# daac-tools/daachorse

Hardware: AMD Instinct MI355X
Metric: haystack GB/s scanned (find_overlapping_iter(..).count(), 100k-pattern bytewise automaton) (higher is better)
Workload: dtype u8/u32 integer

## Files before the change

### daachorse_amd/csrc/gram4_kernels.hip

```cpp
#include <hip/hip_runtime.h>

#include <algorithm>
#include <cstdint>
#include <utility>

#include "device_tables.hpp"
#include "gram4_filter.hpp"
#include "gram4_index.hpp"

namespace daac {

namespace {

typedef uint32_t g4_u32x4_t __attribute__((ext_vector_type(4)));
constexpr uint32_t kList4 = 256;
constexpr uint32_t kProbePercent4 = 3;
typedef __attribute__((address_space(3))) const uint32_t lds4_cu32;
typedef __attribute__((address_space(3))) uint32_t lds4_u32;
typedef __attribute__((address_space(3))) const uint16_t lds4_cu16;
typedef __attribute__((address_space(3))) uint16_t lds4_u16;
typedef __attribute__((address_space(3))) const uint8_t lds4_cu8;
typedef __attribute__((address_space(3))) g4_u32x4_t lds4_u32x4;

__device__ __forceinline__ uint32_t pin4(uint32_t x) {
    asm("" : "+v"(x));
    return x;
}
__device__ __forceinline__ uint32_t mad24(uint32_t a, uint32_t b, uint32_t c) {
    uint32_t d;
    asm("v_mad_u32_u24 %0, %1, %2, %3" : "=v"(d) : "v"(a), "s"(b), "v"(c));
    return d;
}
__device__ __forceinline__ uint32_t wave_shr1_4(uint32_t v, uint32_t lane0) {
    uint32_t d = lane0;
    asm volatile("s_nop 1\nv_mov_b32_dpp %0, %1 wave_shr:1 row_mask:0xf bank_mask:0xf" : "+v"(d) : "v"(v));
    return d;
}
__device__ __forceinline__ uint32_t g4_wave_scan(uint32_t v) {
    v += static_cast<uint32_t>(__builtin_amdgcn_update_dpp(0, static_cast<int>(v), 0x111, 0xf, 0xf, false));
    v += static_cast<uint32_t>(__builtin_amdgcn_update_dpp(0, static_cast<int>(v), 0x112, 0xf, 0xf, false));
    v += static_cast<uint32_t>(__builtin_amdgcn_update_dpp(0, static_cast<int>(v), 0x114, 0xf, 0xf, false));
    v += static_cast<uint32_t>(__builtin_amdgcn_update_dpp(0, static_cast<int>(v), 0x118, 0xf, 0xf, false));
    v += static_cast<uint32_t>(__builtin_amdgcn_update_dpp(0, static_cast<int>(v), 0x142, 0xa, 0xf, false));
    v += static_cast<uint32_t>(__builtin_amdgcn_update_dpp(0, static_cast<int>(v), 0x143, 0xc, 0xf, false));
    return v;
}
template <typename F, int... I>
__device__ __forceinline__ void g4_turns(F &&f, std::integer_sequence<int, I...>) {
    (void)(... && f(std::integral_constant<int, I>{}));
}
__device__ __forceinline__ unsigned long long g4_wave_sum(unsigned long long v) {
#pragma unroll
    for (int off = 32; off > 0; off >>= 1) v += __shfl_down(v, off, 64);
    return v;
}
__device__ __forceinline__ void g4_copy(void *dst, const void *src, uint32_t bytes) {
    const uint4 *s = reinterpret_cast<const uint4 *>(src);
    uint4 *d = reinterpret_cast<uint4 *>(dst);
    for (uint32_t i = threadIdx.x; i < bytes / 16; i += blockDim.x) d[i] = s[i];
}
__device__ __forceinline__ void g4_reduce(unsigned long long cnt, unsigned long long *scratch, unsigned long long *result) {
    const unsigned long long c = g4_wave_sum(cnt);
    __syncthreads();
    const int wave = threadIdx.x >> 6, lane = threadIdx.x & 63;
    if (lane == 0) scratch[wave] = c;
    __syncthreads();
    if (threadIdx.x == 0) {
        unsigned long long r0 = 0;
        for (int w = 0; w < static_cast<int>((blockDim.x + 63) >> 6); ++w) r0 += scratch[w];
        if (r0) atomicAdd(result, r0);
    }
}

}

template <int K, int Q, bool ARITH, int DIR, bool TAIL, bool FILT, bool MPH = false>
__device__ __forceinline__ void gram4_body(const Gram4Dev &g, const GramArgs &a, const Gram4Lds &L, char *smem) {
    static_assert(!(FILT && TAIL), "the filter runs in front of the plain records");
    static_assert(!(FILT && DIR == 0), "the filter's Bloom array lies where the per-word directory would");
    static_assert(!MPH || FILT, "the perfect hash serves the survivors of the filter");
    constexpr int P = 16 * Q;
    constexpr int GS = 8;
    constexpr uint32_t SB = 64u * P;
    constexpr uint32_t SLOT = SB + 32u;
    const uint32_t offM = L.off_m, offS = L.off_s, offC = L.off_cls;
    const uint32_t lo = g.lo, OTH = g.C - 1u, C = g.C;
    auto cls_of = [&](uint32_t byte) -> uint32_t {
        if (ARITH) {
            const uint32_t u = byte - lo;
            return u < OTH ? u : OTH;
        }
        return *reinterpret_cast<lds4_cu8 *>(static_cast<uintptr_t>(offC + byte));
    };
    auto lds_u32 = [&](uint32_t addr) -> uint32_t { return *reinterpret_cast<lds4_cu32 *>(static_cast<uintptr_t>(addr)); };
    auto below = [&](uint32_t k) -> uint32_t { return (1u << k) - 1u; };

    const uint32_t lane = threadIdx.x & 63;
    const uint32_t lane_off = pin4(lane * (16u * Q));
    const uint32_t wave_in_wg = __builtin_amdgcn_readfirstlane(threadIdx.x >> 6);
    const uint32_t C4 = C * 4u, CC4 = C * C * 4u;
    const uint32_t offM1 = g4i_off1(offM, C);
    const uint32_t ub4 = g.unused_byte * 0x01010101u;
    const uint8_t *__restrict__ hay = a.hay_al;
    const uint64_t nwaves = static_cast<uint64_t>(gridDim.x) * (blockDim.x >> 6);
    const uint32_t tb = L.off_wave + wave_in_wg * L.wave_stride;
    const uint32_t listb = wave_in_wg * (kList4 * 2u);
    const uint64_t slab_index = (static_cast<uint64_t>(blockIdx.x) * (blockDim.x >> 6) + wave_in_wg) * a.wq_slab;
    uint4 *__restrict__ slab4 = reinterpret_cast<uint4 *>(a.wq) + slab_index;
    uint32_t wq_n = 0, slab_hi = 0;
    uint64_t epoch_base = 0;
    const uint32_t drain_early = wave_in_wg * 64u;

    unsigned long long tot_cnt = 0;
    uint32_t cnt32 = 0;

    auto load_chunk = [&](uint64_t v) -> uint4 {
        if (v >= a.vlen) return uint4{ub4, ub4, ub4, ub4};
        const g4_u32x4_t q = __builtin_nontemporal_load(reinterpret_cast<const g4_u32x4_t *>(hay + v));
        uint4 r{q.x, q.y, q.z, q.w};
        if (v < a.lead || v + 16 > a.vlen) {
            uint32_t w[4] = {r.x, r.y, r.z, r.w};
            for (int b = 0; b < 16; ++b) {
                const uint64_t p = v + b;
                if (p < a.lead || p >= a.vlen) w[b >> 2] = (w[b >> 2] & ~(0xffu << (8 * (b & 3)))) | (g.unused_byte << (8 * (b & 3)));
            }
            r = uint4{w[0], w[1], w[2], w[3]};
        }
        return r;
    };
    auto raw_at = [&](uint64_t p) -> uint32_t { return (p >= a.lead && p < a.vlen) ? hay[p] : g.unused_byte; };
    auto read_ahead = [&](uint64_t v) -> unsigned long long {
        unsigned long long x;
        if (v >= a.lead && v + 8 <= a.vlen) {
            __builtin_memcpy(&x, hay + v, 8);
        } else {
            x = 0;
            for (int b = 7; b >= 0; --b) x = (x << 8) | ((v + b >= a.lead && v + b < a.vlen) ? hay[v + b] : g.unused_byte);
        }
        return x;
    };
    auto tail_count = [&](const uint4 &rr, unsigned long long text) -> uint32_t {
        const uint32_t edges = rr.x & 15u;
        const unsigned long long path = (static_cast<unsigned long long>(rr.w) << 32) | rr.z;
        const unsigned long long diff = path ^ text;
        uint32_t same = diff ? static_cast<uint32_t>(__builtin_ctzll(diff)) >> 3 : 8u;
        same = same < edges ? same : edges;
        return __popc((rr.x >> 4) & ((2u << same) - 1u) & 0x1ffu);
    };
    auto drain = [&]() {
        const uint4 *__restrict__ recs = TAIL ? g.drec_t : g.drec_c;
        uint32_t n_in = wq_n;
        bool raw = !TAIL;
        while (n_in != 0) {
            uint32_t n_out = 0;
            for (uint32_t base = 0; base < n_in; base += 64u) {
                const uint32_t i = base + lane;
                const bool live = i < n_in;
                uint4 e = uint4{0u, 0u, 0u, 0u};
                if (live) e = slab4[i];
                uint32_t state, n_ahead, pos = e.x;
                unsigned long long ah;
                if (raw) {
                    const uint32_t k1 = cls_of(e.w & 0xffu);
                    state = e.y + __popc(e.x & below(k1));
                    pos = e.z;
                    ah = e.w >> 8;
                    n_ahead = 3;
                } else {
                    state = e.y & 0x07ffffffu;
                    ah = (static_cast<unsigned long long>(e.w & 0xffffffu) << 32) | e.z;
                    n_ahead = e.w >> 24;
                }
                uint4 rr = uint4{0u, 0u, 0u, 0u};
                if (live) rr = recs[state];
                const uint64_t vn = epoch_base + pos + 2;
                bool cont = false;
                uint32_t next_state = 0;
                if (rr.x >> 31) {
                    if (n_ahead < (rr.x & 15u)) ah = read_ahead(vn);
                    cnt32 += tail_count(rr, ah);
                } else {
                    if (live && n_ahead == 0u) { ah = read_ahead(vn); n_ahead = 8; }
                    const uint32_t k = cls_of(static_cast<uint32_t>(ah) & 0xffu);
                    cnt32 += rr.z;
                    cont = ((rr.x >> k) & 1u) != 0;
                    next_state = rr.y + __popc(rr.x & below(k));
                }
                const unsigned long long m = __ballot(cont);
                if (m != 0) {
                    if (cont) {
                        const uint32_t at = n_out + __builtin_amdgcn_mbcnt_hi(static_cast<uint32_t>(m >> 32), __builtin_amdgcn_mbcnt_lo(static_cast<uint32_t>(m), 0));
                        ah >>= 8;
                        slab4[at] = uint4{pos + 1u, next_state, static_cast<uint32_t>(ah), static_cast<uint32_t>(ah >> 32) | ((n_ahead - 1u) << 24)};
                    }
                    n_out += static_cast<uint32_t>(__popcll(m));
                }
            }
            n_in = n_out;
            raw = false;
        }
        wq_n = 0;
    };

    uint32_t q_head = 0, q_tail = 0;
    uint32_t posbias = 0;
    uint32_t st_n = 0;
    uint32_t pend_lo = 0;
    uint4 pend = uint4{0u, 0u, 0u, 0u};
    uint32_t pend_pos = 0;
    uint32_t pend_t0 = 0, pend_t1 = 0;
    bool pend_valid = false;
    uint4 p2 = uint4{0u, 0u, 0u, 0u};
    uint32_t p2_pos = 0, p2_state = 0;
    uint32_t p2_t0 = 0, p2_t1 = 0;
    bool p2_live = false, p2_any = false;
    uint32_t sb_n = 0;
    uint32_t sb_pos = 0, sb_lo = 0, sb_t0 = 0;
    uint32_t fp_pos = 0, fp_t0 = 0;
    const uint32_t offB = L.off_b, bloomW = g.bloom_words;
    auto push_walker = [&](bool go, const uint4 &entry) {
        const unsigned long long m = __ballot(go);
        if (m != 0) {
            if (go) {
                const uint32_t at = wq_n + __builtin_amdgcn_mbcnt_hi(static_cast<uint32_t>(m >> 32), __builtin_amdgcn_mbcnt_lo(static_cast<uint32_t>(m), 0));
                slab4[at] = entry;
            }
            wq_n += __popcll(m);
        }
    };
    auto finish_second = [&]() {
        if (!TAIL || !p2_any) return;
        p2_any = false;
        const uint4 r = p2;
        bool again = false;
        uint32_t st_k = 0, pos = p2_pos, t0 = p2_t0, t1n = (p2_t1 & 0xffffffu) | (7u << 24);
        if (p2_live) {
            if (r.x >> 31) {
                if ((r.x & 15u) <= 7u) cnt32 += tail_count(r, (static_cast<unsigned long long>(p2_t1) << 32) | p2_t0);
                else { again = true; st_k = p2_state; }
            } else {
                cnt32 += r.z;
                const uint32_t k = p2_state >> 27;
                if ((r.x >> k) & 1u) {
                    again = true;
                    const uint32_t k3 = cls_of((p2_t0 >> 8) & 0xffu);
                    st_k = (r.y + __popc(r.x & below(k))) | (k3 << 27);
                    pos = p2_pos + 1u;
                    t0 = __builtin_amdgcn_alignbyte(p2_t1, p2_t0, 1u);
                    t1n = ((p2_t1 >> 8) & 0xffffu) | (6u << 24);
                }
            }
        }
        p2_live = false;
        push_walker(again, uint4{pos, st_k, t0, t1n});
    };
    auto consume_pending = [&]() {
        finish_second();
        if (!pend_valid) return;
        pend_valid = false;
        const uint4 r = pend;
        if (FILT) {
            const uint32_t k1 = cls_of(fp_t0 & 0xffu);
            cnt32 += (r.x >> kGram4EndsBitDev) & 1u;
            push_walker(__builtin_amdgcn_ubfe(r.x, k1, 1) != 0, uint4{r.x, r.y, fp_pos, fp_t0});
            return;
        }
        const uint32_t k1 = cls_of(pend_t0 & 0xffu);
        if (!TAIL) {
            cnt32 += (r.x >> kGram4EndsBitDev) & 1u;
            push_walker(__builtin_amdgcn_ubfe(r.x, k1, 1) != 0, uint4{r.x, r.y, pend_pos, pend_t0});
            return;
        }
        bool go;
        if (r.x >> 31) {
            cnt32 += tail_count(r, (static_cast<unsigned long long>(pend_t1) << 32) | pend_t0);
            go = false;
        } else {
            cnt32 += (r.x >> kGram4EndsBitDev) & 1u;
            go = ((r.x >> k1) & 1u) != 0;
        }
        p2 = uint4{0u, 0u, 0u, 0u};
        p2_live = go;
        p2_any = __ballot(go) != 0;
        if (go) {
            const uint32_t child = r.y + __popc(r.x & below(k1));
            const uint32_t k2 = cls_of((pend_t0 >> 8) & 0xffu);
            p2 = g.drec_t[child];
            p2_pos = pend_pos;
            p2_state = child | (k2 << 27);
            p2_t0 = __builtin_amdgcn_alignbyte(pend_t1, pend_t0, 1u);
            p2_t1 = pend_t1 >> 8;
        }
    };
    auto derive = [&](uint32_t first, uint32_t cnt) {
        if (lane - first < cnt) {
            const uint32_t t3 = *reinterpret_cast<lds4_cu16 *>(static_cast<uintptr_t>(listb + ((q_head + lane - first) << 1)));
            pend_pos = t3 + posbias;
            const uint32_t a0 = t3 & ~3u, sh = t3 & 3u;
            const uint32_t d0 = lds_u32(a0), d1 = lds_u32(a0 + 4u), d2 = lds_u32(a0 + 8u);
            pend_lo = __builtin_amdgcn_alignbyte(d1, d0, sh);
            pend_t0 = __builtin_amdgcn_alignbyte(d2, d1, sh);
            if (TAIL) {
                const uint32_t d3 = lds_u32(a0 + 12u);
                pend_t1 = __builtin_amdgcn_alignbyte(d3, d2, sh);
            }
        }
        q_head += cnt;
    };
    const uint32_t lo_idx = K == 3 ? lo * (C * C + C + 1u) : lo * (C + 1u);
    auto rank_and_ask = [&](uint32_t x_lo) {
        uint32_t idx, d;
        if (ARITH) {
            idx = mad24((x_lo >> 8) & 0xffu, C, ((x_lo >> 16) & 0xffu) - lo_idx);
            if (K == 3) idx = mad24(x_lo & 0xffu, C * C, idx);
            d = (x_lo >> 24) - lo;
        } else {
            const uint32_t c1 = cls_of((x_lo >> 8) & 0xffu), c2 = cls_of((x_lo >> 16) & 0xffu);
            d = cls_of(x_lo >> 24);
            idx = __umul24(c1, C) + c2;
            if (K == 3) idx = __umul24(cls_of(x_lo & 0xffu), C * C) + idx;
        }
        const uint32_t am = (idx << 2) + offM;
        const uint32_t own = lds_u32(am);
        uint32_t rank;
        if (DIR == 0) {
            const uint32_t base = *reinterpret_cast<lds4_cu16 *>(static_cast<uintptr_t>((idx << 1) + offS));
            rank = base + __popc(own & below(d));
        } else {
            const uint32_t grp = am & ~15u;
            const uint32_t qx = lds_u32(grp), qy = lds_u32(grp + 4u), qz = lds_u32(grp + 8u);
            const uint32_t gi = pin4(idx >> 2);
            const uint32_t base = DIR == 1 ? *reinterpret_cast<lds4_cu16 *>(static_cast<uintptr_t>((gi << 1) + offS))
                                           : *reinterpret_cast<lds4_cu32 *>(static_cast<uintptr_t>((gi << 2) + offS));
            const uint32_t mx = static_cast<uint32_t>(__builtin_amdgcn_sbfe(static_cast<int>(0xEEEEEEEEu), idx, 1u));
            const uint32_t my = static_cast<uint32_t>(__builtin_amdgcn_sbfe(static_cast<int>(0xCCCCCCCCu), idx, 1u));
            const uint32_t mz = static_cast<uint32_t>(__builtin_amdgcn_sbfe(static_cast<int>(0x88888888u), idx, 1u));
            uint32_t under = __popc(own & below(d));
            under += __popc(qx & mx & 0x3fffffffu);
            under += __popc(qy & my & 0x3fffffffu);
            under += __popc(qz & mz & 0x3fffffffu);
            rank = base + under;
        }
        if (TAIL) {
            pend = g.dhit_t[rank];
        } else {
            const uint2 h = g.dhit_c[rank];
            pend = uint4{h.x, h.y, 0u, 0u};
        }
    };
    const G4Mph mph = g.mph;
    auto hash_and_ask = [&](uint32_t x_lo) {
        const uint32_t x = K == 3 ? x_lo : x_lo >> 8;
        const uint32_t h = g4f_h(x);
        const uint32_t d = *reinterpret_cast<lds4_cu8 *>(static_cast<uintptr_t>(offS + g4m_bucket(h, mph)));
        const uint2 r = g.dhit_h[g4m_slot(h, g4m_f(x, mph), d, mph)];
        pend = uint4{r.x, r.y, 0u, 0u};
    };
    auto survivors_ask = [&](uint32_t n) {
        consume_pending();
        pend = uint4{0u, 0u, 0u, 0u};
        if (lane < n) { if constexpr (MPH) hash_and_ask(sb_lo); else rank_and_ask(sb_lo); }
        fp_pos = sb_pos;
        fp_t0 = lane < n ? sb_t0 : 0u;
        pend_valid = true;
    };
    auto process_batch = [&](uint32_t n) {
        __builtin_amdgcn_s_setprio(2);
        if (FILT) {
            derive(st_n, n - st_n);
            st_n = 0;
            const G4Probe pr = g4f_probe(K == 3 ? pend_lo : pend_lo >> 8, pend_t0 & 0xffu, bloomW);
            const uint32_t fw = lds_u32(offB + (pr.word << 2));
            const unsigned long long in_batch = n >= 64u ? ~0ull : (1ull << n) - 1ull;
            const unsigned long long pm = (__builtin_amdgcn_ballot_w64((pr.go & ~fw) == 0u) | __builtin_amdgcn_ballot_w64((pr.ends & ~fw) == 0u)) & in_batch;
            if (pm != 0) {
                const uint32_t s = static_cast<uint32_t>(__popcll(pm));
                const uint32_t r = __builtin_amdgcn_mbcnt_hi(static_cast<uint32_t>(pm >> 32), __builtin_amdgcn_mbcnt_lo(static_cast<uint32_t>(pm), 0));
                uint32_t t;
                asm("v_cndmask_b32_e64 %0, 63, %1, %2" : "=v"(t) : "v"(r), "s"(pm));
                const uint32_t tgt = ((t + sb_n) << 2) & 0xfcu;
                const uint32_t r_pos = static_cast<uint32_t>(__builtin_amdgcn_ds_permute(static_cast<int>(tgt), static_cast<int>(pend_pos)));
                const uint32_t r_lo = static_cast<uint32_t>(__builtin_amdgcn_ds_permute(static_cast<int>(tgt), static_cast<int>(pend_lo)));
                const uint32_t r_t0 = static_cast<uint32_t>(__builtin_amdgcn_ds_permute(static_cast<int>(tgt), static_cast<int>(pend_t0)));
                const bool mine = lane - sb_n < s;
                sb_pos = mine ? r_pos : sb_pos;
                sb_lo = mine ? r_lo : sb_lo;
                sb_t0 = mine ? r_t0 : sb_t0;
                if (sb_n + s >= 64u) {
                    survivors_ask(64u);
                    sb_pos = r_pos; sb_lo = r_lo; sb_t0 = r_t0;
                    sb_n = sb_n + s - 64u;
                } else {
                    sb_n += s;
                }
            }
            return;
        }
        consume_pending();
        derive(st_n, n - st_n);
        st_n = 0;
        pend = uint4{0u, 0u, 0u, 0u};
        if (lane < n) {
            rank_and_ask(pend_lo);
        } else {
            pend_t0 = 0;
            pend_t1 = 0;
        }
        pend_valid = true;
    };

    uint64_t region = static_cast<uint64_t>(blockIdx.x) * (blockDim.x >> 6) + wave_in_wg;
    while (region < a.nregions) {
      slab_hi = static_cast<uint32_t>((region * a.region_bytes) >> 31);
      epoch_base = static_cast<uint64_t>(slab_hi) << 31;
      for (; region < a.nregions && static_cast<uint32_t>((region * a.region_bytes) >> 31) == slab_hi; region += nwaves) {
        const uint64_t rbase = region * a.region_bytes;
        const uint64_t rend = rbase + a.region_bytes < a.vlen ? rbase + a.region_bytes : a.vlen;
        uint32_t carry = 0, tail4 = 0;
#pragma unroll
        for (int i = 0; i < K; ++i) carry |= (rbase >= static_cast<uint64_t>(K - i) ? cls_of(raw_at(rbase - (K - i))) : OTH) << (8 * i);
#pragma unroll
        for (int i = 0; i < 4; ++i) tail4 |= (rbase >= static_cast<uint64_t>(4 - i) ? raw_at(rbase - (4 - i)) : static_cast<uint32_t>(g.unused_byte)) << (8 * i);
        tail4 = __builtin_amdgcn_readfirstlane(tail4);
        carry = __builtin_amdgcn_readfirstlane(carry);
        uint32_t mcarry;
        {
            uint32_t x = (((carry >> (8 * (K - 1))) & 0xffu) << 2) + offM;
            x += __umul24((carry >> (8 * (K - 2))) & 0xffu, C4);
            if (K == 3) x += __umul24(carry & 0xffu, CC4);
            mcarry = __builtin_amdgcn_readfirstlane(lds_u32(x));
        }

        const uint32_t rlen = static_cast<uint32_t>(rend - rbase);
        const uint32_t fast_lo = rbase < 16u ? SB : 0u;
        const uint32_t fast_hi = rlen & ~(SB - 1u);
        auto fetch = [&](uint32_t off, uint4 (&out)[Q]) {
            if (off >= fast_lo && off < fast_hi) {
                const uint8_t *__restrict__ base = hay + rbase + off;
                uint32_t voff = lane_off;
                asm volatile("" : "+v"(voff));
#pragma unroll
                for (int q = 0; q < Q; ++q) {
                    const g4_u32x4_t t = __builtin_nontemporal_load(reinterpret_cast<const g4_u32x4_t *>(base + voff + 16u * q));
                    out[q] = uint4{t.x, t.y, t.z, t.w};
                }
                return;
            }
            const uint64_t s0 = rbase + off;
#pragma unroll
            for (int q = 0; q < Q; ++q) out[q] = uint4{ub4, ub4, ub4, ub4};
            if (off < rlen) {
#pragma unroll
                for (int q = 0; q < Q; ++q) out[q] = load_chunk(s0 + lane * P + 16u * q);
            } else if (lane == 0 && off < rlen + SB) {
                out[0] = load_chunk(s0);
            }
        };
        uint4 pf0[Q], pf1[Q];
        fetch(0u, pf0);
        fetch(SB, pf1);
        const uint32_t rbias = static_cast<uint32_t>(rbase - epoch_base) - (tb + 16u - 3u);

        for (uint32_t off = 0; off < rlen; off += SB) {
            if (wq_n + 64u * P + 128u + drain_early > a.wq_slab) drain();
            uint4 cur[Q];
#pragma unroll
            for (int q = 0; q < Q; ++q) { cur[q] = pf0[q]; pf0[q] = pf1[q]; }
            consume_pending();
            __builtin_amdgcn_s_setprio(0);
            fetch(off + 2u * SB, pf1);

            if (q_tail != q_head) {
                const uint32_t n_left = q_tail - q_head;
                derive(st_n, n_left);
                st_n += n_left;
            }
            q_head = q_tail = 0;
            const uint32_t slot = tb;
            const uint32_t my_text = slot + 16u + lane * P;
            posbias = rbias + off;
#pragma unroll
            for (int q = 0; q < Q; ++q)
                *reinterpret_cast<lds4_u32x4 *>(static_cast<uintptr_t>(my_text + 16u * q)) = g4_u32x4_t{cur[q].x, cur[q].y, cur[q].z, cur[q].w};
            if (lane == 0) {
                *reinterpret_cast<lds4_u32 *>(static_cast<uintptr_t>(slot + 12u)) = tail4;
                *reinterpret_cast<lds4_u32x4 *>(static_cast<uintptr_t>(slot + 16u + SB)) = g4_u32x4_t{pf0[0].x, pf0[0].y, pf0[0].z, pf0[0].w};
            }
            tail4 = __builtin_amdgcn_readlane(cur[Q - 1].w, 63);

            uint32_t kx[K + P];
#pragma unroll
            for (int q = 0; q < Q; ++q) {
                const uint32_t w[4] = {cur[q].x, cur[q].y, cur[q].z, cur[q].w};
#pragma unroll
                for (int b = 0; b < 16; ++b) {
                    kx[K + 16 * q + b] = pin4(cls_of((w[b >> 2] >> (8 * (b & 3))) & 0xffu));
                    __builtin_assume(kx[K + 16 * q + b] < 32u);
                }
            }
            uint32_t pk = 0;
#pragma unroll
            for (int i = 0; i < K; ++i) pk |= kx[P + i] << (8 * i);
            const uint32_t left = wave_shr1_4(pk, carry);
            carry = __builtin_amdgcn_readlane(pk, 63);
#pragma unroll
            for (int i = 0; i < K; ++i) { kx[i] = (left >> (8 * i)) & 0xffu; __builtin_assume(kx[i] < 32u); }

            uint32_t H = 0, ccnt = cnt32, roll = 0, mprev = 0;
#pragma unroll
            for (int grp = 0; grp < P / GS; ++grp) {
                uint32_t mw[GS];
                uint32_t qe = 0;
#pragma unroll
                for (int jj = 0; jj < GS; ++jj) {
                    const int j = grp * GS + jj;
                    uint32_t x;
                    if (K == 3 && (jj & 1)) {
                        x = g4i_odd(qe, kx[K + j], offM1, C);
                    } else if (K == 3) {
                        const G4Idx e = g4i_even(kx[K + j], kx[K + j - 1], kx[K + j - 2], offM, C);
                        x = e.addr;
                        qe = e.q;
                    } else {
                        x = pin4((kx[K + j] << 2) + offM);
                        x = mad24(kx[K + j - 1], C4, x);
                    }
                    mw[jj] = lds_u32(x);
                }
#pragma unroll
                for (int jj = 0; jj < GS; ++jj) {
                    const int j = grp * GS + jj;
                    roll = __builtin_amdgcn_alignbit(roll, mw[jj], 30);
                    if (j > 0) H = __builtin_amdgcn_alignbit((jj == 0 ? mprev : mw[jj - 1]) >> kx[K + j], H, 1);
                    if ((j & 15) == 15) {
                        ccnt = pin4(__popc(roll) + ccnt);
                        ccnt = pin4(__popc(roll & 0xaaaaaaaau) + ccnt);
                        roll = 0;
                    }
                }
                mprev = mw[GS - 1];
            }
            {
                const uint32_t mleft = wave_shr1_4(mprev, mcarry);
                mcarry = __builtin_amdgcn_readlane(mprev, 63);
                H |= __builtin_amdgcn_ubfe(mleft, kx[K], 1) << (32 - P);
            }
            cnt32 = ccnt;

            static_assert(P == 16 * Q, "lane_off = lane * 16 Q is this lane's offset in the step: my_text = tb + 16 + lane_off");
            const uint32_t text_adj = tb + (lane_off - (32u - P) + 13u);
            for (;;) {
                if (__ballot(H != 0u) == 0) break;
                const uint32_t n = __popc(H);
                const uint32_t incl = g4_wave_scan(n);
                const uint32_t tot = __builtin_amdgcn_readlane(incl, 63);
                const uint32_t first = q_tail + incl - n;
                const uint32_t room = first < kList4 ? kList4 - first : 0u;
                const uint32_t lim = n < room ? n : room;
                const uint32_t at = pin4(listb + (first << 1));
                g4_turns([&](auto tc) -> bool {
                    constexpr uint32_t t = decltype(tc)::value;
                    const bool w = t < lim;
                    if (__ballot(w) == 0) return false;
                    if (w) {
                        *reinterpret_cast<lds4_u16 *>(static_cast<uintptr_t>(at + 2u * t)) = static_cast<uint16_t>(text_adj + __builtin_ctz(H));
                        H &= H - 1u;
                    }
                    return true;
                }, std::make_integer_sequence<int, P>{});
                const uint32_t in = std::min(tot, kList4 - q_tail);
                q_tail += in;
                while (st_n + q_tail - q_head >= 64u) process_batch(64u);
                if (in == tot) break;
                const uint32_t n_left = q_tail - q_head;
                if (lane < n_left) {
                    const uint16_t v = *reinterpret_cast<lds4_cu16 *>(static_cast<uintptr_t>(listb + ((q_head + lane) << 1)));
                    *reinterpret_cast<lds4_u16 *>(static_cast<uintptr_t>(listb + (lane << 1))) = v;
                }
                q_head = 0;
                q_tail = n_left;
            }
        }
        tot_cnt += cnt32;
        cnt32 = 0;
      }
      if (st_n + q_tail - q_head != 0) process_batch(st_n + q_tail - q_head);
      if (FILT && sb_n != 0) { survivors_ask(sb_n); sb_n = 0; }
      consume_pending();
      finish_second();
      drain();
      tot_cnt += cnt32;
      cnt32 = 0;
    }
    g4_reduce(tot_cnt, reinterpret_cast<unsigned long long *>(smem), a.result);
}

template <int K, int Q, bool ARITH, int DIR, int TPB, bool FILT, bool MPH = false>
__global__ __launch_bounds__(TPB) void gram4_kernel(const Gram4Dev g, const GramArgs a, const Gram4Lds L) {
    extern __shared__ __attribute__((aligned(16))) char smem[];
    constexpr int DIRC = DIR == 0 ? 1 : DIR;
    if (!ARITH) g4_copy(smem + L.off_cls, g.cls, 256);
    g4_copy(smem + L.off_m, g.m, g.m_bytes);
    uint32_t *votes = reinterpret_cast<uint32_t *>(smem + L.off_wave);
    if (threadIdx.x == 0) *votes = 0;
    __syncthreads();
    if (__builtin_amdgcn_groupstaticsize() != 0) __builtin_trap();
    bool tail = a.sel_want == 1u;
    if (a.sel_want == 2u) {
        const uint64_t span = a.vlen > a.lead + 16 ? a.vlen - a.lead - 8 : 0;
        bool go = false;
        if (span != 0) {
            unsigned long long h = (static_cast<unsigned long long>(threadIdx.x) + 1) * 0x9E3779B97F4A7C15ull;
            h ^= h >> 29;
            const uint64_t p = a.lead + 3 + (h % (span - 3));
            const uint8_t *t = a.hay_al + p;
            const uint32_t OTH = g.C - 1u;
            auto cl = [&](uint32_t b) -> uint32_t {
                if (ARITH) { const uint32_t u = b - g.lo; return u < OTH ? u : OTH; }
                return reinterpret_cast<const uint8_t *>(smem + L.off_cls)[b];
            };
            const uint32_t *m = reinterpret_cast<const uint32_t *>(smem + L.off_m);
            const uint32_t c0 = cl(t[-3]), c1 = cl(t[-2]), c2 = cl(t[-1]), d = cl(t[0]), k1 = cl(t[1]);
            const uint32_t ctx = K == 3 ? (c0 * g.C + c1) * g.C + c2 : c1 * g.C + c2;
            const uint32_t w = m[ctx];
            if ((w >> d) & 1u & (d < OTH ? 1u : 0u)) {
                uint32_t rank = __popc(w & ((1u << d) - 1u));
                for (uint32_t j = ctx & ~3u; j < ctx; ++j) rank += __popc(m[j] & 0x3fffffffu);
                rank += g.s16 ? reinterpret_cast<const uint16_t *>(g.sdir)[ctx >> 2] : reinterpret_cast<const uint32_t *>(g.sdir)[ctx >> 2];
                const uint2 r = g.dhit_c[rank];
                go = ((r.x >> k1) & 1u) != 0;
            }
        }
        const unsigned long long bm = __ballot(go);
        if ((threadIdx.x & 63) == 0 && bm != 0) atomicAdd(votes, static_cast<uint32_t>(__popcll(bm)));
        __syncthreads();
        tail = *votes * 100u > static_cast<uint32_t>(TPB) * kProbePercent4;
        __syncthreads();
    }
    if (FILT && !tail) {
        g4_copy(smem + L.off_s, MPH ? static_cast<const void *>(g.mph_disp) : g.sdir, L.s_bytes_f);
        g4_copy(smem + L.off_b, g.bloom, g.bloom_words * 4u);
    } else {
        g4_copy(smem + L.off_s, DIR == 0 ? static_cast<const void *>(g.rfull) : g.sdir, L.s_bytes);
    }
    __syncthreads();
    if (tail) gram4_body<K, Q, ARITH, DIR, true, false>(g, a, L, smem);
    else if constexpr (FILT) gram4_body<K, Q, ARITH, DIRC, false, true, MPH>(g, a, L, smem);
    else gram4_body<K, Q, ARITH, DIR, false, false>(g, a, L, smem);
}

template <int K, int Q, bool ARITH, int DIR, int TPB, bool FILT, bool MPH = false>
static hipError_t launch4_inst(const Gram4Dev &dev, const GramArgs &a, const Gram4Lds &L, uint32_t blocks, hipStream_t stream) {
    const hipError_t e = hipFuncSetAttribute(reinterpret_cast<const void *>(gram4_kernel<K, Q, ARITH, DIR, TPB, FILT, MPH>),
                                             hipFuncAttributeMaxDynamicSharedMemorySize, static_cast<int>(L.lds_bytes));
    if (e != hipSuccess) return e;
    hipLaunchKernelGGL((gram4_kernel<K, Q, ARITH, DIR, TPB, FILT, MPH>), dim3(blocks), dim3(TPB), L.lds_bytes, stream, dev, a, L);
    return hipGetLastError();
}
template <int K, int Q, int TPB, bool ARITH>
static hipError_t launch4_d(const Gram4Dev &dev, const GramArgs &a, const Gram4Lds &L, uint32_t blocks, hipStream_t stream) {
    if (L.filter && L.mph) {
        if (L.dir == 0) return launch4_inst<K, Q, ARITH, 0, TPB, true, true>(dev, a, L, blocks, stream);
        if (L.dir == 1) return launch4_inst<K, Q, ARITH, 1, TPB, true, true>(dev, a, L, blocks, stream);
        return launch4_inst<K, Q, ARITH, 2, TPB, true, true>(dev, a, L, blocks, stream);
    }
    if (L.filter) {
        if (L.dir == 0) return launch4_inst<K, Q, ARITH, 0, TPB, true>(dev, a, L, blocks, stream);
        if (L.dir == 1) return launch4_inst<K, Q, ARITH, 1, TPB, true>(dev, a, L, blocks, stream);
        return launch4_inst<K, Q, ARITH, 2, TPB, true>(dev, a, L, blocks, stream);
    }
    if (L.dir == 0) return launch4_inst<K, Q, ARITH, 0, TPB, false>(dev, a, L, blocks, stream);
    if (L.dir == 1) return launch4_inst<K, Q, ARITH, 1, TPB, false>(dev, a, L, blocks, stream);
    return launch4_inst<K, Q, ARITH, 2, TPB, false>(dev, a, L, blocks, stream);
}
template <int K, int Q, int TPB>
static hipError_t launch4_k(const Gram4Dev &dev, const GramArgs &a, const Gram4Lds &L, uint32_t blocks, hipStream_t stream) {
    return L.arith ? launch4_d<K, Q, TPB, true>(dev, a, L, blocks, stream) : launch4_d<K, Q, TPB, false>(dev, a, L, blocks, stream);
}

bool gram4_plan(const Gram4Dev &dev, uint32_t ppl, uint32_t waves, bool rfull, bool want_arith, bool want_filter, uint32_t lds_limit, Gram4Lds &L) {
    L = Gram4Lds{};
    if (rfull && dev.rfull == nullptr) return false;
    const uint32_t slot = 64u * ppl + 32u;
    L.wave_stride = slot;
    L.off_wave = waves * kList4 * 2u;
    L.threads = waves * 64u;
    L.arith = (want_arith && dev.arith) ? 1u : 0u;
    const uint32_t per_wg = L.off_wave + waves * L.wave_stride;
    L.off_cls = per_wg;
    L.off_s = per_wg + (L.arith ? 0u : 256u);
    L.dir = rfull ? 0u : (dev.s16 ? 1u : 2u);
    L.s_bytes = rfull ? dev.rfull_bytes : dev.s_bytes;
    uint32_t region = L.s_bytes;
    if (want_filter && dev.bloom != nullptr) {
        const uint32_t front = dev.mph_disp != nullptr ? dev.mph_bytes : dev.s_bytes;
        const uint32_t with = front + dev.bloom_words * 4u;
        if (L.off_s + std::max(region, with) + dev.m_bytes <= lds_limit) {
            L.filter = 1u;
            L.mph = dev.mph_disp != nullptr ? 1u : 0u;
            L.s_bytes_f = front;
            L.off_b = L.off_s + front;
            region = std::max(region, with);
        }
    }
    L.off_m = L.off_s + region;
    L.lds_bytes = L.off_m + dev.m_bytes;
    return L.lds_bytes <= lds_limit;
}
uint32_t gram4_filter_room(uint32_t m_bytes, uint32_t sdir_bytes, bool arith, uint32_t lds_limit) {
    const uint32_t fixed = 16u * kList4 * 2u + 16u * (64u * 32u + 32u) + (arith ? 0u : 256u) + sdir_bytes + m_bytes;
    return fixed < lds_limit ? (lds_limit - fixed) & ~15u : 0u;
}

hipError_t launch_gram4_scan(const Gram4Dev &dev, const GramArgs &a, const Gram4Lds &L, uint32_t blocks, hipStream_t stream) {
    if (a.ppl == 32 && L.threads == 1024)
        return dev.K == 3 ? launch4_k<3, 2, 1024>(dev, a, L, blocks, stream) : launch4_k<2, 2, 1024>(dev, a, L, blocks, stream);
    if (a.ppl == 32)
        return dev.K == 3 ? launch4_k<3, 2, 512>(dev, a, L, blocks, stream) : launch4_k<2, 2, 512>(dev, a, L, blocks, stream);
    if (L.threads == 512)
        return dev.K == 3 ? launch4_k<3, 1, 512>(dev, a, L, blocks, stream) : launch4_k<2, 1, 512>(dev, a, L, blocks, stream);
    return dev.K == 3 ? launch4_k<3, 1, 1024>(dev, a, L, blocks, stream) : launch4_k<2, 1, 1024>(dev, a, L, blocks, stream);
}

}
```

Baseline: 1775.

## Drain work queue incrementally with batched multi-row loads and cooked-entry tagging

The drain routine now processes up to DR batches of 64 queue entries at once (three when Q==2), issuing all slab and record loads before consuming them so the memory latencies overlap. In non-tail mode it drains one pass early once the queue passes a per-wave threshold, keeping the sub-64 remainder. Raw and already-advanced entries can now sit in the same queue, so advanced ones are tagged with a high bit in the state word. The intent is to keep the queue short and hide drain latency, at the cost of more drain calls, higher register pressure and more interleaving with the main scan.

```diff
diff --git a/daachorse_amd/csrc/gram4_kernels.hip b/daachorse_amd/csrc/gram4_kernels.hip
--- a/daachorse_amd/csrc/gram4_kernels.hip
+++ b/daachorse_amd/csrc/gram4_kernels.hip
@@ -15,6 +15,7 @@
 typedef uint32_t g4_u32x4_t __attribute__((ext_vector_type(4)));
 constexpr uint32_t kList4 = 256;
 constexpr uint32_t kProbePercent4 = 3;
+constexpr uint32_t kG4Cooked = 1u << 31;
 typedef __attribute__((address_space(3))) const uint32_t lds4_cu32;
 typedef __attribute__((address_space(3))) uint32_t lds4_u32;
 typedef __attribute__((address_space(3))) const uint16_t lds4_cu16;
@@ -81,6 +82,7 @@
     static_assert(!MPH || FILT, "the perfect hash serves the survivors of the filter");
     constexpr int P = 16 * Q;
     constexpr int GS = 8;
+    constexpr int DR = Q == 2 ? 3 : 1;
     constexpr uint32_t SB = 64u * P;
     constexpr uint32_t SLOT = SB + 32u;
     const uint32_t offM = L.off_m, offS = L.off_s, offC = L.off_cls;
@@ -109,7 +111,8 @@
     uint4 *__restrict__ slab4 = reinterpret_cast<uint4 *>(a.wq) + slab_index;
     uint32_t wq_n = 0, slab_hi = 0;
     uint64_t epoch_base = 0;
-    const uint32_t drain_early = wave_in_wg * 64u;
+    const uint32_t drain_at = 64u * DR + wave_in_wg * 16u;
+    const uint32_t drain_early = TAIL ? wave_in_wg * 64u : 0u;
 
     unsigned long long tot_cnt = 0;
     uint32_t cnt32 = 0;
@@ -147,59 +150,68 @@
         same = same < edges ? same : edges;
         return __popc((rr.x >> 4) & ((2u << same) - 1u) & 0x1ffu);
     };
-    auto drain = [&]() {
+    auto drain = [&](bool to_empty) {
         const uint4 *__restrict__ recs = TAIL ? g.drec_t : g.drec_c;
-        uint32_t n_in = wq_n;
-        bool raw = !TAIL;
-        while (n_in != 0) {
-            uint32_t n_out = 0;
-            for (uint32_t base = 0; base < n_in; base += 64u) {
-                const uint32_t i = base + lane;
-                const bool live = i < n_in;
-                uint4 e = uint4{0u, 0u, 0u, 0u};
-                if (live) e = slab4[i];
-                uint32_t state, n_ahead, pos = e.x;
-                unsigned long long ah;
-                if (raw) {
-                    const uint32_t k1 = cls_of(e.w & 0xffu);
-                    state = e.y + __popc(e.x & below(k1));
-                    pos = e.z;
-                    ah = e.w >> 8;
-                    n_ahead = 3;
-                } else {
-                    state = e.y & 0x07ffffffu;
-                    ah = (static_cast<unsigned long long>(e.w & 0xffffffu) << 32) | e.z;
-                    n_ahead = e.w >> 24;
-                }
-                uint4 rr = uint4{0u, 0u, 0u, 0u};
-                if (live) rr = recs[state];
-                const uint64_t vn = epoch_base + pos + 2;
-                bool cont = false;
-                uint32_t next_state = 0;
-                if (rr.x >> 31) {
-                    if (n_ahead < (rr.x & 15u)) ah = read_ahead(vn);
-                    cnt32 += tail_count(rr, ah);
-                } else {
-                    if (live && n_ahead == 0u) { ah = read_ahead(vn); n_ahead = 8; }
-                    const uint32_t k = cls_of(static_cast<uint32_t>(ah) & 0xffu);
-                    cnt32 += rr.z;
-                    cont = ((rr.x >> k) & 1u) != 0;
-                    next_state = rr.y + __popc(rr.x & below(k));
-                }
-                const unsigned long long m = __ballot(cont);
-                if (m != 0) {
-                    if (cont) {
-                        const uint32_t at = n_out + __builtin_amdgcn_mbcnt_hi(static_cast<uint32_t>(m >> 32), __builtin_amdgcn_mbcnt_lo(static_cast<uint32_t>(m), 0));
-                        ah >>= 8;
-                        slab4[at] = uint4{pos + 1u, next_state, static_cast<uint32_t>(ah), static_cast<uint32_t>(ah >> 32) | ((n_ahead - 1u) << 24)};
+        const uint32_t keep = to_empty ? 0u : wq_n & 63u;
+        do {
+            const uint32_t n_in = wq_n;
+            uint32_t n_out = keep;
+            for (uint32_t base = keep; base < n_in; base += 64u * DR) {
+                uint4 e[DR], rr[DR];
+                uint32_t pos[DR], n_ahead[DR];
+                unsigned long long ah[DR];
+#pragma unroll
+                for (int j = 0; j < DR; ++j) {
+                    const uint32_t i = base + 64u * j + lane;
+                    e[j] = uint4{0u, 0u, 0u, 0u};
+                    if (i < n_in) e[j] = slab4[i];
+                }
+#pragma unroll
+                for (int j = 0; j < DR; ++j) {
+                    const bool live = base + 64u * j + lane < n_in;
+                    const bool raw = !TAIL && (e[j].y & kG4Cooked) == 0u;
+                    uint32_t state = e[j].y & 0x07ffffffu;
+                    pos[j] = e[j].x;
+                    ah[j] = (static_cast<unsigned long long>(e[j].w & 0xffffffu) << 32) | e[j].z;
+                    n_ahead[j] = e[j].w >> 24;
+                    if (!TAIL) {
+                        const uint32_t k1 = cls_of(e[j].w & 0xffu);
+                        state = raw ? e[j].y + __popc(e[j].x & below(k1)) : state;
+                        pos[j] = raw ? e[j].z : pos[j];
+                        ah[j] = raw ? static_cast<unsigned long long>(e[j].w >> 8) : ah[j];
+                        n_ahead[j] = raw ? 3u : n_ahead[j];
                     }
-                    n_out += static_cast<uint32_t>(__popcll(m));
-                }
-            }
-            n_in = n_out;
-            raw = false;
-        }
-        wq_n = 0;
+                    rr[j] = uint4{0u, 0u, 0u, 0u};
+                    if (live) rr[j] = recs[state];
+                    if (live && n_ahead[j] == 0u) { ah[j] = read_ahead(epoch_base + pos[j] + 2); n_ahead[j] = 8; }
+                }
+#pragma unroll
+                for (int j = 0; j < DR; ++j) {
+                    bool cont = false;
+                    uint32_t next_state = 0;
+                    if (rr[j].x >> 31) {
+                        if (n_ahead[j] < (rr[j].x & 15u)) ah[j] = read_ahead(epoch_base + pos[j] + 2);
+                        cnt32 += tail_count(rr[j], ah[j]);
+                    } else {
+                        const uint32_t k = cls_of(static_cast<uint32_t>(ah[j]) & 0xffu);
+                        cnt32 += rr[j].z;
+                        cont = ((rr[j].x >> k) & 1u) != 0;
+                        next_state = rr[j].y + __popc(rr[j].x & below(k));
+                    }
+                    const unsigned long long m = __ballot(cont);
+                    if (m != 0) {
+                        if (cont) {
+                            const uint32_t at = n_out + __builtin_amdgcn_mbcnt_hi(static_cast<uint32_t>(m >> 32), __builtin_amdgcn_mbcnt_lo(static_cast<uint32_t>(m), 0));
+                            const unsigned long long rest = ah[j] >> 8;
+                            slab4[at] = uint4{pos[j] + 1u, next_state | (TAIL ? 0u : kG4Cooked), static_cast<uint32_t>(rest),
+                                              static_cast<uint32_t>(rest >> 32) | ((n_ahead[j] - 1u) << 24)};
+                        }
+                        n_out += static_cast<uint32_t>(__popcll(m));
+                    }
+                }
+            }
+            wq_n = n_out;
+        } while (to_empty && wq_n != 0);
     };
 
     uint32_t q_head = 0, q_tail = 0;
@@ -462,7 +474,10 @@
         const uint32_t rbias = static_cast<uint32_t>(rbase - epoch_base) - (tb + 16u - 3u);
 
         for (uint32_t off = 0; off < rlen; off += SB) {
-            if (wq_n + 64u * P + 128u + drain_early > a.wq_slab) drain();
+            {
+                const bool no_room = wq_n + 64u * P + 128u + drain_early > a.wq_slab;
+                if (no_room || (!TAIL && wq_n >= drain_at)) drain(no_room);
+            }
             uint4 cur[Q];
 #pragma unroll
             for (int q = 0; q < Q; ++q) { cur[q] = pf0[q]; pf0[q] = pf1[q]; }
@@ -588,7 +603,7 @@
       if (FILT && sb_n != 0) { survivors_ask(sb_n); sb_n = 0; }
       consume_pending();
       finish_second();
-      drain();
+      drain(true);
       tot_cnt += cnt32;
       cnt32 = 0;
     }
```

Result: no change. 1779 (median of 6 runs) (+0.2%).
